# PolyChord/PolyChordLite

Measured on AMD Instinct MI355X. Metric: likelihood evals/sec, 20D Gaussian nlive=2000, higher is better.
Workload: dtype f64; 1 GPU; configs[1]: 20-D Gaussian, nlive=2000, num_repeats=40, one full run per step; batch_chains=1000, parallelism=repeat-sharded x1, mode=one run at a time per GPU; R runs in step: roofline.in_step

## Files before the change

polychordlite_amd/csrc/pc_update.hip:

```cpp
#include "pc_state.h"
#include "pc_launch.h"
#include "pc_upd_flag.h"
#include <atomic>
#include <cstdio>
#include <cstdlib>


__device__ __forceinline__ void upd_stage_masked(const double *src0, unsigned long long mask, unsigned long long mmask, double *dst,
                                                 double *tile, int TS, const double *sh, int D, int nT, int lane)
{
    const int ne = dst ? nT : D + 1;
    int n = 0;
    while (mask) {
        int idx[16], cnt = 0;
#pragma unroll
        for (int u = 0; u < 16; ++u) {
            idx[u] = 0;
            if (mask) { idx[u] = __ffsll((long long)mask) - 1; mask &= mask - 1; cnt = u + 1; }
        }
        for (int e = lane; e < ne; e += 64) {
            double v[16];
#pragma unroll
            for (int u = 0; u < 16; ++u) if (u < cnt) v[u] = (e < nT) ? src0[(size_t)idx[u] * nT + e] : 0.0;
            if (dst) {
#pragma unroll
                for (int u = 0; u < 16; ++u) if (u < cnt) dst[(size_t)(n + u) * nT + e] = v[u];
            }
            if (e <= D) {
                const double s = e < D ? sh[e] : 0.0;
#pragma unroll
                for (int u = 0; u < 16; ++u)
                    if (u < cnt && ((mmask >> idx[u]) & 1ull))
                        tile[(size_t)__popcll(mmask & ((1ull << idx[u]) - 1ull)) * TS + e] = e < D ? v[u] - s : 1.0;
            }
        }
        n += cnt;
    }
}

__global__ __launch_bounds__(UPD_NT) void k_upd_flag(PcState S, int nph, unsigned char *keep, int *blk_count, int def, int nblk) { upd_flag_body<false>(S, nph, keep, blk_count, def, nblk, (int)blockIdx.x * 4 + (int)(threadIdx.x >> 6)); }
__global__ __launch_bounds__(UPD_NT) void k_upd_flag_many(const PcManyRec *R, int def) { const PcManyView r = pc_many_view(R, blockIdx.y); if ((int)blockIdx.x * 4 >= r.ia[PC_REC_I_BLOCKS]) return; upd_flag_body<false>(r.S, r.ia[PC_REC_I_ROWS], (unsigned char *)r.p[PC_REC_KEEP], (int *)r.p[PC_REC_BLK], def, r.ia[PC_REC_I_BLOCKS], (int)blockIdx.x * 4 + (int)(threadIdx.x >> 6)); }

__device__ __forceinline__ bool upd_ticket_last(int *ctr, int n, int *last_s)
{
    asm volatile("s_waitcnt vmcnt(0)" ::: "memory");
    __syncthreads();
    if (threadIdx.x == 0) {
        const int t = __hip_atomic_fetch_add(ctr, 1, __ATOMIC_RELAXED, __HIP_MEMORY_SCOPE_AGENT);
        const int last = t == n - 1;
        if (last) {
            __builtin_amdgcn_fence(__ATOMIC_ACQUIRE, "agent");
            asm volatile("s_waitcnt vmcnt(0)" ::: "memory");
            __hip_atomic_store(ctr, 0, __ATOMIC_RELAXED, __HIP_MEMORY_SCOPE_AGENT);
        }
        *last_s = last;
    }
    __syncthreads();
    return *last_s != 0;
}
#define UPD_TICKET_FLAG 1
#define UPD_TICKET_FINAL 2
#define UPD_TICKET_GROUP 16

#define UPD_SELF_BLOCKS 4096
__global__ __launch_bounds__(UPD_NT) void k_upd_flag_scan(PcState S, int nph, unsigned char *keep, int *blk, int def, int nblk, int *ctr)
{
    __shared__ int last_s, wsum[4];
    upd_flag_body<false>(S, nph, keep, blk, def, nblk, (int)blockIdx.x * 4 + (int)(threadIdx.x >> 6));
    if (!upd_ticket_last(ctr + UPD_TICKET_FLAG, (int)gridDim.x, &last_s)) return;
    const int tid = threadIdx.x, lane = tid & 63, wv = tid >> 6, i0 = 16 * tid;
    int c[16], s = 0;
#pragma unroll
    for (int u = 0; u < 16; ++u) { c[u] = (i0 + u < nblk) ? blk[i0 + u] : 0; s += c[u]; }
    int inc = s;
#pragma unroll
    for (int o = 1; o < 64; o <<= 1) { const int t = __shfl_up(inc, o); if (lane >= o) inc += t; }
    if (lane == 63) wsum[wv] = inc;
    __syncthreads();
    int run = inc - s;
    for (int x = 0; x < wv; ++x) run += wsum[x];
#pragma unroll
    for (int u = 0; u < 16; ++u) { if (i0 + u < nblk) blk[i0 + u] = run; run += c[u]; }
    if (tid == UPD_NT - 1) ctr[0] = run;
}


__global__ __launch_bounds__(1024) void k_upd_scan(int *cnt, int n, int *total)
{
    __shared__ int wsum[16];
    __shared__ int carry_s;
    const int tid = threadIdx.x, lane = tid & 63, wv = tid >> 6;
    int carry = 0;
    for (int base = 0; base < n; base += 4096) {
        const int i0 = base + 4 * tid;
        int c[4];
#pragma unroll
        for (int u = 0; u < 4; ++u) c[u] = (i0 + u < n) ? cnt[i0 + u] : 0;
        const int s = (c[0] + c[1]) + (c[2] + c[3]);
        int inc = s;
#pragma unroll
        for (int o = 1; o < 64; o <<= 1) { const int t = __shfl_up(inc, o); if (lane >= o) inc += t; }
        if (lane == 63) wsum[wv] = inc;
        __syncthreads();
        int pre = carry;
        for (int x = 0; x < wv; ++x) pre += wsum[x];
        int run = pre + inc - s;
#pragma unroll
        for (int u = 0; u < 4; ++u) { if (i0 + u < n) cnt[i0 + u] = run; run += c[u]; }
        if (tid == 1023) carry_s = pre + inc;
        __syncthreads();
        carry = carry_s;
    }
    if (tid == 0) *total = carry;
}

__global__ __launch_bounds__(UPD_NT) void k_upd_index(int nph, const unsigned char *keep, const int *blk_off, int *idx)
{
    __shared__ int cnt[4];
    const int tid = threadIdx.x, lane = tid & 63, wv = tid >> 6;
    const int j = blockIdx.x * UPD_ROWS + tid;
    const bool km = j < nph && (keep[j] & 2);
    const unsigned long long m = __ballot(km);
    if (lane == 0) cnt[wv] = __popcll(m);
    __syncthreads();
    int off = blk_off[blockIdx.x];
    for (int x = 0; x < wv; ++x) off += cnt[x];
    if (km) idx[off + __popcll(m & ((1ull << lane) - 1ull))] = j;
}

#define UPD_IDX_NT 256
#define UPD_IDX_BLOCKS 16
__device__ __forceinline__ void upd_index_self_body(int nph, const unsigned char *keep, const int *blk_count, int nblk, int *idx, int *total)
{
    __shared__ int part[4];
    const int tid = threadIdx.x, lane = tid & 63, wv = tid >> 6;
    const int sb0 = blockIdx.x * UPD_IDX_BLOCKS;
    int s = 0;
    for (int b = tid; b < sb0; b += UPD_IDX_NT) s += blk_count[b];
#pragma unroll
    for (int o = 32; o >= 1; o >>= 1) s += __shfl_xor(s, o);
    if (lane == 0) part[wv] = s;
    __syncthreads();
    int off = (part[0] + part[1]) + (part[2] + part[3]);
    const int sbw = sb0 + 4 * wv;
    for (int x = sb0; x < sbw && x < nblk; ++x) off += blk_count[x];
    const unsigned long long below = (1ull << lane) - 1ull;
    for (int q = 0; q < 4; ++q) {
        const int sb = sbw + q;
        if (sb >= nblk) return;
        const int j0 = sb * UPD_ROWS + 4 * lane;
        unsigned w = 0;
        if (j0 + 3 < nph) w = *(const unsigned *)(keep + j0);
        else for (int u = 0; u < 4; ++u) if (j0 + u < nph) w |= (unsigned)keep[j0 + u] << (8 * u);
        int pos = off, all = 0;
        bool f[4];
#pragma unroll
        for (int u = 0; u < 4; ++u) {
            f[u] = (w >> (8 * u + 1)) & 1u;
            const unsigned long long m = __ballot(f[u]);
            pos += __popcll(m & below); all += __popcll(m);
        }
#pragma unroll
        for (int u = 0; u < 4; ++u) if (f[u]) { idx[pos] = j0 + u; pos++; }
        off += all;
        if (sb == nblk - 1 && lane == 0) *total = off;
    }
}
__global__ __launch_bounds__(UPD_IDX_NT) void k_upd_index_self(int nph, const unsigned char *keep, const int *blk_count, int nblk, int *idx, int *total) { upd_index_self_body(nph, keep, blk_count, nblk, idx, total); }
__global__ __launch_bounds__(UPD_IDX_NT) void k_upd_index_self_many(const PcManyRec *R) { const PcManyView r = pc_many_view(R, blockIdx.y); if ((int)blockIdx.x * 16 >= r.ia[PC_REC_I_BLOCKS]) return; upd_index_self_body(r.ia[PC_REC_I_ROWS], (const unsigned char *)r.p[PC_REC_KEEP], (const int *)r.p[PC_REC_BLK], r.ia[PC_REC_I_BLOCKS], (int *)r.p[PC_REC_PHC2], (int *)r.p[PC_REC_TOTAL]); }


__device__ __forceinline__ void upd_stage_idx(const double *base, const int *ridx, int cnt, double *tile, int TS, const double *sh, int D, int nT, int lane)
{
    if (cnt <= 0) return;
    int idx[16];
#pragma unroll
    for (int u = 0; u < 16; ++u) idx[u] = u < cnt ? ridx[u] : 0;
    for (int e0 = lane; e0 <= D; e0 += 128) {
        const int e1 = e0 + 64;
        double v0[16], v1[16];
#pragma unroll
        for (int u = 0; u < 16; ++u) if (u < cnt) { v0[u] = e0 < D ? base[(size_t)idx[u] * nT + e0] : 1.0; v1[u] = e1 < D ? base[(size_t)idx[u] * nT + e1] : 1.0; }
        const double s0 = e0 < D ? sh[e0] : 0.0, s1 = e1 < D ? sh[e1] : 0.0;
#pragma unroll
        for (int u = 0; u < 16; ++u) if (u < cnt) { tile[(size_t)u * TS + e0] = v0[u] - s0; if (e1 <= D) tile[(size_t)u * TS + e1] = v1[u] - s1; }
    }
}

#define UPD_FOLD 16
__device__ __forceinline__ void upd_fold_body(const double *part, int nb, int E, double *part2, int g)
{
    for (int e = threadIdx.x; e < E; e += 256) {
        double t[UPD_FOLD];
#pragma unroll
        for (int u = 0; u < UPD_FOLD; ++u) t[u] = (g * UPD_FOLD + u < nb) ? part[(size_t)(g * UPD_FOLD + u) * E + e] : 0.0;
        double s = 0.0;
#pragma unroll
        for (int u = 0; u < UPD_FOLD; ++u) s += t[u];
        upd_store_wt(part2 + (size_t)g * E + e, s);
    }
}
__global__ __launch_bounds__(256) void k_upd_fold(const double *part, int nb, int E, double *part2) { upd_fold_body(part, nb, E, part2, blockIdx.x); }
__global__ __launch_bounds__(256) void k_upd_fold_many(const PcManyRec *R, int nb, int E) { double *part = pc_as_global((double *)R[blockIdx.y].p[PC_REC_PART], R); upd_fold_body(part, nb, E, part + (size_t)nb * E, blockIdx.x); }


__device__ __forceinline__ void upd_final_fold(int nb, const double *part, int E, int nE, double *tot)
{
    for (int e = threadIdx.x; e < nE; e += 256) {
        double s[4] = {0.0, 0.0, 0.0, 0.0};
        for (int k0 = 0; k0 < nb; k0 += 4 * 16) {
            double t[4][16];
#pragma unroll
            for (int h = 0; h < 4; ++h)
#pragma unroll
                for (int u = 0; u < 16; ++u) t[h][u] = (k0 + h + 4 * u < nb) ? part[(size_t)(k0 + h + 4 * u) * E + e] : 0.0;
#pragma unroll
            for (int h = 0; h < 4; ++h)
#pragma unroll
                for (int u = 0; u < 16; ++u) s[h] += t[h][u];
        }
        tot[e] = (s[0] + s[1]) + (s[2] + s[3]);
    }
    __syncthreads();
}
#define UPD_FINAL_LDS (544 + 1024 + 1024 + 32 + 1)
template <int DMAX>
__device__ __forceinline__ void upd_final_stage(const PcState &S, double *lds, double *shift, int def)
{
    double *tot = lds, *A = tot + 544, *L = A + 1024, *mu = L + 1024;
    int *bad = (int *)(mu + 32);
    const int tid = threadIdx.x, D = S.D, npair = D * (D + 1) / 2;
#ifdef UPD_DBG
    const long long f0 = clock64();
#endif
    if (tid == 0) *bad = 0;
    const double n = tot[npair + D];
    if (tid < D) mu[tid] = tot[npair + tid] / n;
    __syncthreads();
    for (int p = tid; p < D * D; p += 256) {
        const int a = p / D, b = p % D, lo = a < b ? a : b, hi = a < b ? b : a;
        const int idx = lo * D - lo * (lo - 1) / 2 + (hi - lo);
        const double c = n > 1.0 ? tot[idx] / n - mu[lo] * mu[hi] : 0.0;
        A[p] = c; L[p] = 0.0;
        S.cov[p] = c;
    }
    __syncthreads();
#ifdef UPD_DBG
    const long long f1 = clock64();
#endif
    if (tid < 64) {
        double a[DMAX];
#pragma unroll
        for (int k = 0; k < DMAX; ++k) a[k] = (tid < D && k < D) ? A[tid * D + k] : 0.0;
        bool fail = false;
#pragma unroll
        for (int i = 0; i < DMAX; ++i) {
            if (i < D && !fail) {
                const double aii = readlane_f64(a[i], i);
                if (aii <= 0.0) fail = true;
                else {
                    const double lii = sqrt(aii);
                    const double lji = (tid == i) ? lii : a[i] / lii;
                    if (tid >= i) a[i] = lji;
#pragma unroll
                    for (int k = i + 1; k < DMAX; ++k) { const double lki = readlane_f64(lji, k); if (tid > i) a[k] -= lji * lki; }
                }
            }
        }
        if (fail) { if (tid == 0) *bad = 1; }
        else if (tid < D) {
#pragma unroll
            for (int k = 0; k < DMAX; ++k) if (k < D) L[tid * D + k] = (k <= tid) ? a[k] : 0.0;
        }
    }
    __syncthreads();
    if (*bad) {
        double tr = 0.0;
        for (int k = 0; k < D; ++k) tr += A[k * D + k];
        for (int p = tid; p < D * D; p += 256) L[p] = (p / D == p % D) ? sqrt(tr) : 0.0;
        __syncthreads();
    }
    for (int p = tid; p < D * D; p += 256) S.chol[p] = L[p];
    if (tid < D) shift[tid] += mu[tid];
    if (tid == 0) { if (!(def && S.ctl->upd_keep_thr)) S.death_thr[0] = -PC_HUGE; if (def) S.ctl->upd_pending = 0; }
#ifdef UPD_DBG
    if (tid == 0) { const long long f2 = clock64(); S.ctl->gen_cyc[2] += f1 - f0; S.ctl->gen_cyc[3] += f2 - f1; S.ctl->nn_walks += f0; }
#endif
}
template <int NT>
__device__ __forceinline__ void upd_final_body(const PcState &S, int nb, const double *part, int E, double *lds, double *shift, int def)
{
    const int D = S.D;
    upd_final_fold(nb, part, E, D * (D + 1) / 2 + D + 1, lds);
    if (NT != 2 && D <= 8) upd_final_stage<8>(S, lds, shift, def);
    else if (D <= 16) upd_final_stage<16>(S, lds, shift, def);
    else if (NT != 1 && D <= 24) upd_final_stage<24>(S, lds, shift, def);
    else if (NT != 1) upd_final_stage<32>(S, lds, shift, def);
}
__global__ __launch_bounds__(256) void k_upd_final(PcState S, int nb, const double *part, int E, double *shift, int def) { __shared__ double lds[UPD_FINAL_LDS]; upd_final_body<0>(S, nb, part, E, lds, shift, def); }
__global__ __launch_bounds__(256) void k_upd_final_many(const PcManyRec *R, int nb, int E, int def, int G) { __shared__ double lds[UPD_FINAL_LDS]; const PcManyView r = pc_many_view(R, blockIdx.y); upd_final_body<0>(r.S, nb, (const double *)r.p[PC_REC_PART] + (size_t)G * E, E, lds, (double *)r.p[PC_REC_SHIFT], def); }


typedef double upd_v4d __attribute__((ext_vector_type(4)));
template <int NT, int W>
__device__ __forceinline__ void updg_accumulate(const double *tile, int TS, int n16, int wv, int li, int lk, upd_v4d (&acc)[(NT <= 2) ? NT * (NT + 1) / 2 : (NT * (NT + 1) / 2 + 3) / 4])
{
    if constexpr (NT <= 2) {
        for (int q0 = 4 * wv; q0 < n16; q0 += 16) {
            const double *row = tile + (size_t)(q0 + lk) * TS + li;
            double x[NT];
#pragma unroll
            for (int t = 0; t < NT; ++t) x[t] = row[16 * t];
            int q = 0;
#pragma unroll
            for (int ti = 0; ti < NT; ++ti)
#pragma unroll
                for (int tj = ti; tj < NT; ++tj, ++q) acc[q] = __builtin_amdgcn_mfma_f64_16x16x4f64(x[ti], x[tj], acc[q], 0, 0, 0);
        }
    } else {
        for (int ks = 0; ks < (n16 >> 2); ++ks) {
            const double *row = tile + (size_t)(4 * ks + lk) * TS + li;
            double x[NT];
#pragma unroll
            for (int t = 0; t < NT; ++t) x[t] = row[16 * t];
            int q = 0;
#pragma unroll
            for (int ti = 0; ti < NT; ++ti)
#pragma unroll
                for (int tj = ti; tj < NT; ++tj, ++q)
                    if ((q & 3) == W) acc[q >> 2] = __builtin_amdgcn_mfma_f64_16x16x4f64(x[ti], x[tj], acc[q >> 2], 0, 0, 0);
        }
    }
}
__device__ __forceinline__ int updg_slot(int D, int ti, int tj, int li, int lk, int r)
{
    const int a = 16 * ti + lk + 4 * r, b = 16 * tj + li, npair = D * (D + 1) / 2;
    if (a > b || b > D) return -1;
    return (b < D) ? a * D - a * (a - 1) / 2 + (b - a) : (a < D ? npair + a : npair + D);
}

template <int NT, bool IDX, bool CHAIN>
__device__ __forceinline__ void upd_gather_body(const PcState &S, int nph, int nblk, const unsigned char *keep, const int *blk_off,
                                                double *ph2, double *phL2, unsigned *phC2, unsigned long long *phU2,
                                                const int *idx, const int *nidx_p,
                                                const double *shift, double *part, int E, int def, int nlb, int ndb, double *shift_out = nullptr, int *ctr = nullptr)
{
    static_assert(!CHAIN || IDX, "the chain is pool mode's");
    extern __shared__ __attribute__((aligned(16))) char smem[];
    constexpr bool KS = NT <= 2;
    constexpr int TS = KS ? 16 * NT + 1 : 16 * NT + ((NT & 1) ? 0 : 16);
    constexpr int CAP = KS ? 128 : 64;
    constexpr int NACC = KS ? NT * (NT + 1) / 2 : (NT * (NT + 1) / 2 + 3) / 4;
    __shared__ unsigned long long m64[4], mm64[4];
    __shared__ int dix[256];
    const int tmark = def ? S.ctl->upd_tmark : 0x7fffffff, nph0u = def ? S.ctl->upd_nph0 : 0x7fffffff, updT = def ? S.ctl->upd_T : 0;
    const int tid = threadIdx.x, lane = tid & 63, wv = tid >> 6, li = lane & 15, lk = lane >> 4, D = S.D, nT = S.nT;
    constexpr bool pool = IDX;
    double *tile = (double *)smem;
    double *sh = tile + (size_t)CAP * TS;
    for (int d = tid; d < D; d += 256) sh[d] = shift[d];
    for (int e = tid; e < CAP * TS; e += 256) tile[e] = 0.0;
    upd_v4d acc[NACC];
#pragma unroll
    for (int t = 0; t < NACC; ++t) acc[t] = upd_v4d{0.0, 0.0, 0.0, 0.0};
    int nfill = 0;
#ifdef UPD_DBG
    const long long g0 = clock64();
#endif
    auto flush = [&]() __attribute__((always_inline)) {
        __syncthreads();
        const int n16 = (nfill + 15) & ~15;
        for (int e = tid; e < (n16 - nfill) * (D + 1); e += 256) tile[(size_t)(nfill + e / (D + 1)) * TS + e % (D + 1)] = 0.0;
        __syncthreads();
        if (KS || wv == 0) updg_accumulate<NT, 0>(tile, TS, n16, wv, li, lk, acc);
        else if (wv == 1) updg_accumulate<NT, 1>(tile, TS, n16, wv, li, lk, acc);
        else if (wv == 2) updg_accumulate<NT, 2>(tile, TS, n16, wv, li, lk, acc);
        else updg_accumulate<NT, 3>(tile, TS, n16, wv, li, lk, acc);
        __syncthreads();
        nfill = 0;
    };
    auto piece = [&](const double *src, int sub, double *dst) __attribute__((always_inline)) {
        const unsigned long long ms = m64[sub], mms = mm64[sub], below = (1ull << (16 * wv)) - 1ull;
        const int cnt = __popcll(mms);
        if (cnt == 0 && (dst == nullptr || ms == 0ull)) return;
        if (nfill + cnt > CAP) flush();
        upd_stage_masked(src + (size_t)(sub * 64 + 16 * wv) * nT, ((dst ? ms : mms) >> (16 * wv)) & 0xFFFFull, (mms >> (16 * wv)) & 0xFFFFull,
                         dst ? dst + (size_t)__popcll(ms & below) * nT : nullptr, tile + (size_t)(nfill + __popcll(mms & below)) * TS, TS, sh, D, nT, lane);
        nfill += cnt;
    };
    if constexpr (IDX) {
        const int nidx = *nidx_p;
        const int gchunk = (int)gridDim.x - nlb - ndb;
        if constexpr (CHAIN) {
            __shared__ int off_s[UPD_SELF_BLOCKS + 1], ridx_s[2][64];
            const bool mine = (int)blockIdx.x < gchunk && (int)blockIdx.x * 64 < nidx;
            if (mine) {
                for (int b = tid; b < nblk; b += 256) off_s[b] = blk_off[b];
                if (tid == 0) off_s[nblk] = nidx;
                __syncthreads();
            }
            const unsigned long long below = (1ull << lane) - 1ull;
            int par = 0;
            for (int c = blockIdx.x; mine && c * 64 < nidx; c += gchunk, par ^= 1) {
                const int p0 = c * 64, have = min(64, nidx - p0), p1 = p0 + have;
                if (nfill + have > CAP) flush();
                int lo = 0, hi = nblk - 1;
                while (lo < hi) { const int mid = (lo + hi + 1) >> 1; if (off_s[mid] <= p0) lo = mid; else hi = mid - 1; }
                for (int sb = lo + wv; sb < nblk; sb += 4) {
                    const int o = off_s[sb];
                    if (o >= p1) break;
                    if (off_s[sb + 1] == o) continue;
                    const int j0 = sb * UPD_ROWS + 4 * lane;
                    unsigned w = 0;
                    if (j0 + 3 < nph) w = *(const unsigned *)(keep + j0);
                    else for (int u = 0; u < 4; ++u) if (j0 + u < nph) w |= (unsigned)keep[j0 + u] << (8 * u);
                    int pos = o;
                    bool f[4];
#pragma unroll
                    for (int u = 0; u < 4; ++u) { f[u] = (w >> (8 * u + 1)) & 1u; pos += __popcll(__ballot(f[u]) & below); }
#pragma unroll
                    for (int u = 0; u < 4; ++u) if (f[u]) { if (pos >= p0 && pos < p1) ridx_s[par][pos - p0] = j0 + u; pos++; }
                }
                __syncthreads();
                upd_stage_idx(S.phantom, ridx_s[par] + 16 * wv, min(16, have - 16 * wv), tile + (size_t)(nfill + 16 * wv) * TS, TS, sh, D, nT, lane);
                nfill += have;
            }
        } else
        for (int c = blockIdx.x; (int)blockIdx.x < gchunk && c * 64 < nidx; c += gchunk) {
            const int have = min(64, nidx - c * 64);
            if (nfill + have > CAP) flush();
            upd_stage_idx(S.phantom, idx + c * 64 + 16 * wv, min(16, have - 16 * wv), tile + (size_t)(nfill + 16 * wv) * TS, TS, sh, D, nT, lane);
            nfill += have;
        }
    }
    const int total = nblk + nlb + ndb;
    for (int b = IDX ? ((int)blockIdx.x >= (int)gridDim.x - nlb - ndb ? nblk + (int)blockIdx.x - ((int)gridDim.x - nlb - ndb) : total) : blockIdx.x; b < total; b += gridDim.x) {
        __syncthreads();
        if (b < nblk) {
            const int j = b * 256 + tid;
            const bool k = (j < nph) && keep[j];
            const bool km = k && (j < nph0u || (pool ? updT - 1 - (j - nph0u) / S.nr : (j - nph0u) / S.nr) < tmark);
            const unsigned long long m = __ballot(k), mm = __ballot(km);
            if (lane == 0) { m64[wv] = m; mm64[wv] = mm; }
            __syncthreads();
            int off = 0;
            if (!pool) {
                off = blk_off[b];
                for (int x = 0; x < wv; ++x) off += __popcll(m64[x]);
                if (k) {
                    const int pos = off + __popcll(m & ((1ull << lane) - 1ull));
                    phL2[pos] = S.ph_logL[j]; phC2[pos] = S.ph_cuid[j]; phU2[pos] = S.ph_uid[j];
                }
                off = blk_off[b];
            }
            const double *src = S.phantom + (size_t)b * 256 * nT;
            for (int sub = 0; sub < 4; ++sub) {
                piece(src, sub, pool ? nullptr : ph2 + (size_t)off * nT);
                off += __popcll(m64[sub]);
            }
        } else if (b < nblk + nlb) {
            const int r0 = (b - nblk) * 256, r = r0 + tid;
            const bool k = (r < S.Ncap) && S.live_cluster[r] == 0 && (!def || S.slot_step[r] < tmark);
            const unsigned long long m = __ballot(k);
            if (lane == 0) { m64[wv] = m; mm64[wv] = m; }
            __syncthreads();
            const double *src = S.live + (size_t)r0 * nT;
            for (int sub = 0; sub < 4; ++sub) piece(src, sub, nullptr);
        } else {
            const PcCtl *ctl = S.ctl;
            const int T = ctl->upd_T, ts = ctl->upd_ts;
            const int t = tmark + (b - nblk - nlb) * 256 + tid;
            int di = -1;
            if (t < ts) {
                const PcPlan *pw = S.plan + (T - 1 - t);
                const int src = pw->dead_src;
                const bool existed = src >= 0 || (T - 1 - (-src - 1)) < tmark;
                if (pw->dead_idx >= 0 && pw->logw > S.logzero && existed) di = pw->dead_idx;
            }
            const unsigned long long m = __ballot(di >= 0);
            if (di >= 0) dix[wv * 64 + __popcll(m & ((1ull << lane) - 1ull))] = (int)di;
            if (lane == 0) m64[wv] = m;
            __syncthreads();
            for (int sub = 0; sub < 4; ++sub) {
                const int cnt = __popcll(m64[sub]);
                if (cnt == 0) continue;
                if (nfill + cnt > CAP) flush();
                upd_stage_idx(S.dead, dix + sub * 64 + 16 * wv, min(16, cnt - 16 * wv), tile + (size_t)(nfill + 16 * wv) * TS, TS, sh, D, nT, lane);
                nfill += cnt;
            }
        }
    }
#ifdef UPD_DBG
    const long long g1 = clock64();
#endif
    flush();
    double *out = part + (size_t)blockIdx.x * E;
    if constexpr (KS) {
        double *wres = tile;
#pragma unroll
        for (int t = 0; t < NACC; ++t)
#pragma unroll
            for (int r = 0; r < 4; ++r) wres[((size_t)wv * NACC + t) * 256 + (lk + 4 * r) * 16 + li] = acc[t][r];
        __syncthreads();
        if (wv == 0) {
            int q = 0;
#pragma unroll
            for (int ti = 0; ti < NT; ++ti)
#pragma unroll
                for (int tj = ti; tj < NT; ++tj, ++q)
#pragma unroll
                    for (int r = 0; r < 4; ++r) {
                        const int p = updg_slot(D, ti, tj, li, lk, r), idx = (lk + 4 * r) * 16 + li;
                        if (p >= 0) upd_store_wt(out + p, (wres[(size_t)(0 * NACC + q) * 256 + idx] + wres[(size_t)(1 * NACC + q) * 256 + idx]) +
                                              (wres[(size_t)(2 * NACC + q) * 256 + idx] + wres[(size_t)(3 * NACC + q) * 256 + idx]));
                    }
        }
    } else {
        int q = 0;
#pragma unroll
        for (int ti = 0; ti < NT; ++ti)
#pragma unroll
            for (int tj = ti; tj < NT; ++tj, ++q)
                if ((q & 3) == wv) {
#pragma unroll
                    for (int r = 0; r < 4; ++r) { const int p = updg_slot(D, ti, tj, li, lk, r); if (p >= 0) out[p] = acc[q >> 2][r]; }
                }
    }
#ifdef UPD_DBG
    if (IDX && tid == 0) {
        const int gch = (int)gridDim.x - nlb - ndb, kind = (int)blockIdx.x < gch ? 0 : ((int)blockIdx.x < gch + nlb ? 1 : 2);
        atomicAdd((unsigned long long *)&S.ctl->wave_cyc[kind], (unsigned long long)(g1 - g0));
        atomicAdd((unsigned long long *)&S.ctl->wave_cyc[3], (unsigned long long)(clock64() - g1));
    }
#endif
    if constexpr (CHAIN && KS) {
        static_assert(sizeof(double) * UPD_FINAL_LDS <= sizeof(double) * 4 * 3 * 256, "the final stage's LDS fits the row tile");
        __shared__ int last_s;
        const int G = gridDim.x, g = blockIdx.x / UPD_FOLD, ng = (G + UPD_FOLD - 1) / UPD_FOLD;
        double *part2 = part + (size_t)G * E;
        if (!upd_ticket_last(ctr + UPD_TICKET_GROUP + g, min(UPD_FOLD, G - g * UPD_FOLD), &last_s)) return;
        upd_fold_body(part, G, E, part2, g);
        if (!upd_ticket_last(ctr + UPD_TICKET_FINAL, ng, &last_s)) return;
        upd_final_body<NT>(S, ng, part2, E, tile, shift_out, def);
    }
}
template <int NT, bool IDX>
__global__ __launch_bounds__(256) void k_upd_gather(PcState S, int nph, int nblk, const unsigned char *keep, const int *blk_off,
                                                    double *ph2, double *phL2, unsigned *phC2, unsigned long long *phU2,
                                                    const int *idx, const int *nidx_p,
                                                    const double *shift, double *part, int E, int def, int nlb, int ndb)
{ upd_gather_body<NT, IDX, false>(S, nph, nblk, keep, blk_off, ph2, phL2, phC2, phU2, idx, nidx_p, shift, part, E, def, nlb, ndb); }
template <int NT>
__global__ __launch_bounds__(256) void k_upd_chain(PcState S, int nph, int nblk, const unsigned char *keep, const int *blk_off, double *shift, double *part, int E, int def, int nlb, int ndb, int *ctr)
{ upd_gather_body<NT, true, true>(S, nph, nblk, keep, blk_off, nullptr, nullptr, nullptr, nullptr, nullptr, ctr, shift, part, E, def, nlb, ndb, shift, ctr); }
template <int NT>
__global__ __launch_bounds__(256) void k_upd_gather_many(const PcManyRec *R, int E, int def, int nlb, int ndb)
{
    const PcManyView r = pc_many_view(R, blockIdx.y);
    upd_gather_body<NT, true, false>(r.S, r.ia[PC_REC_I_ROWS], r.ia[PC_REC_I_BLOCKS], (const unsigned char *)r.p[PC_REC_KEEP], (const int *)r.p[PC_REC_BLK], (double *)r.p[PC_REC_PH2], (double *)r.p[PC_REC_PHL2], (unsigned *)r.p[PC_REC_PHC2],
                              (unsigned long long *)r.p[PC_REC_PHU2], (const int *)r.p[PC_REC_PHC2], (const int *)r.p[PC_REC_TOTAL], (const double *)r.p[PC_REC_SHIFT], (double *)r.p[PC_REC_PART], E, def, nlb, ndb);
}


__global__ __launch_bounds__(1024) void k_upd_final_w(PcState S, int nb, const double *part, int E, double *shift, int def, double *ncov, int *count)
{
    extern __shared__ __attribute__((aligned(16))) char smem[];
    double *tot = (double *)smem;
    __shared__ double mu[128];
    const int tid = threadIdx.x, D = S.D, npair = D * (D + 1) / 2, nE = npair + D + 1;
    for (int e = tid; e < nE; e += 1024) {
        double s = 0.0;
        for (int k = 0; k < nb; k += 8) {
            double t[8];
#pragma unroll
            for (int u = 0; u < 8; ++u) t[u] = (k + u < nb) ? part[(size_t)(k + u) * E + e] : 0.0;
#pragma unroll
            for (int u = 0; u < 8; ++u) s += t[u];
        }
        tot[e] = s;
    }
    __syncthreads();
    const double n = tot[npair + D];
    if (tid < D) mu[tid] = tot[npair + tid] / n;
    __syncthreads();
    for (int p = tid; p < D * D; p += 1024) {
        const int a = p / D, b = p % D, lo = a < b ? a : b, hi = a < b ? b : a;
        ncov[p] = n > 1.0 ? tot[lo * D - lo * (lo - 1) / 2 + (hi - lo)] - n * mu[lo] * mu[hi] : 0.0;
    }
    if (tid < D) shift[tid] += mu[tid];
    if (tid == 0) { count[0] = (int)n; if (!(def && S.ctl->upd_keep_thr)) S.death_thr[0] = -PC_HUGE; if (def) S.ctl->upd_pending = 0; }
}

static int upd_grid(const PcState *S, int nph, int deferred)
{
    const int nblk = (nph + UPD_ROWS - 1) / UPD_ROWS, nlb = (S->Ncap + UPD_ROWS - 1) / UPD_ROWS, ndb = deferred ? (S->B + UPD_ROWS - 1) / UPD_ROWS : 0;
    static const int cap_env = std::getenv("PC_UPD_GRID") ? std::atoi(std::getenv("PC_UPD_GRID")) : 0;
    const int cap = cap_env > 0 ? cap_env : (S->D < 32 ? 384 : 512);
    if (S->pool) { const int nch = (nph + 63) / 64; return (nch < cap ? (nch > 0 ? nch : 1) : cap) + nlb + ndb; }
    const int total = nblk + nlb + ndb;
    return total < cap ? total : cap;
}

extern "C" int pc_update_fused_ok(const PcState *S, int nc) { return nc == 1 && S->D <= 128; }
extern "C" int pc_update_fused_blocks(const PcState *S, int nph)
{
    const int G = upd_grid(S, nph, 1), E = pc_update_fused_entries(S);
    return G + (G + UPD_FOLD - 1) / UPD_FOLD + (S->D * S->D + 2 + E - 1) / E;
}
extern "C" int pc_update_fused_entries(const PcState *S) { const int e = S->D * (S->D + 1) / 2 + S->D + 1; return (e + 31) & ~31; }

extern "C" void pc_launch_update_fused(const PcState *S, int nph, unsigned char *keep, int *blk, int *d_total, double *ph2, double *phL2,
                                       unsigned *phC2, unsigned long long *phU2, double *part, double *shift, int deferred, hipStream_t st)
{
    pc_launch_update_fused_at(S, nph, keep, blk, d_total, ph2, phL2, phC2, phU2, part, shift, deferred, 0, st);
}
extern "C" void pc_launch_update_fused_at(const PcState *S, int nph, unsigned char *keep, int *blk, int *d_total, double *ph2, double *phL2,
                                          unsigned *phC2, unsigned long long *phU2, double *part, double *shift, int deferred, int flagged, hipStream_t st)
{
    const int D = S->D, nblk = (nph + UPD_ROWS - 1) / UPD_ROWS, nlb = (S->Ncap + UPD_ROWS - 1) / UPD_ROWS, E = pc_update_fused_entries(S);
    const int ndb = deferred ? (S->B + UPD_ROWS - 1) / UPD_ROWS : 0;
    const int NTv = (D + 1 + 15) / 16, TSv = NTv <= 2 ? 16 * NTv + 1 : 16 * NTv + ((NTv & 1) ? 0 : 16), CAPv = NTv <= 2 ? 128 : 64;
    const int G = upd_grid(S, nph, deferred), ng = (G + UPD_FOLD - 1) / UPD_FOLD;
    double *part2 = part + (size_t)G * E;
    size_t shw = sizeof(double) * ((size_t)CAPv * TSv + D);
    if (NTv <= 2 && shw < sizeof(double) * (size_t)(4 * 3 * 256)) shw = sizeof(double) * (size_t)(4 * 3 * 256);
    if (S->pool && nblk <= UPD_SELF_BLOCKS && UPD_TICKET_GROUP + ng <= PC_UPD_CTR_INTS && (S->ablate & PC_ABL_UPDATE_CHAIN)) {
        int *ctr = d_total;
        hipLaunchKernelGGL(k_upd_flag_scan, dim3((nblk + 3) / 4), dim3(UPD_NT), 0, st, *S, nph, keep, blk, deferred, nblk, ctr);
#define UPDC_LAUNCH(NT) { \
        pc_need_dyn_lds((const void *)k_upd_chain<NT>, shw); \
        hipLaunchKernelGGL((k_upd_chain<NT>), dim3(G), dim3(256), shw, st, *S, nph, nblk, (const unsigned char *)keep, (const int *)blk, shift, part, E, deferred, nlb, ndb, ctr); }
        switch (NTv) { case 1: UPDC_LAUNCH(1) break; case 2: UPDC_LAUNCH(2) break; case 3: UPDC_LAUNCH(3) break; case 4: UPDC_LAUNCH(4) break;
                       case 5: UPDC_LAUNCH(5) break; case 6: UPDC_LAUNCH(6) break; case 7: UPDC_LAUNCH(7) break; case 8: UPDC_LAUNCH(8) break;
                       default: UPDC_LAUNCH(9) break; }
#undef UPDC_LAUNCH
        if (D < 32) return;
    } else {
        if (!(flagged && S->pool && deferred)) hipLaunchKernelGGL(k_upd_flag, dim3((nblk + 3) / 4), dim3(UPD_NT), 0, st, *S, nph, keep, blk, deferred, nblk);
        if (!S->pool) pc_launch_scan_blocks(blk, nblk, d_total, &S->ctl->nphantom, st);
        else if (nblk <= UPD_SELF_BLOCKS && !std::getenv("PC_UPD_SCAN_LAUNCH"))
            hipLaunchKernelGGL(k_upd_index_self, dim3((nblk + 15) / 16), dim3(UPD_IDX_NT), 0, st, nph, (const unsigned char *)keep, (const int *)blk, nblk, (int *)phC2, d_total);
        else {
            hipLaunchKernelGGL(k_upd_scan, dim3(1), dim3(1024), 0, st, blk, nblk, d_total);
            hipLaunchKernelGGL(k_upd_index, dim3(nblk), dim3(UPD_NT), 0, st, nph, (const unsigned char *)keep, (const int *)blk, (int *)phC2);
        }
        int devi = 0; (void)hipGetDevice(&devi); devi &= 63;
#define UPDG_LAUNCH(NT) { \
            pc_need_dyn_lds((const void *)k_upd_gather<NT, false>, shw); \
                              pc_need_dyn_lds((const void *)k_upd_gather<NT, true>, shw); \
             \
            if (S->pool) hipLaunchKernelGGL((k_upd_gather<NT, true>), dim3(G), dim3(256), shw, st, *S, nph, nblk, (const unsigned char *)keep, (const int *)blk, \
                               ph2, phL2, phC2, phU2, (const int *)phC2, (const int *)d_total, (const double *)shift, part, E, deferred, nlb, ndb); \
            else hipLaunchKernelGGL((k_upd_gather<NT, false>), dim3(G), dim3(256), shw, st, *S, nph, nblk, (const unsigned char *)keep, (const int *)blk, \
                               ph2, phL2, phC2, phU2, (const int *)nullptr, (const int *)nullptr, (const double *)shift, part, E, deferred, nlb, ndb); }
        switch (NTv) { case 1: UPDG_LAUNCH(1) break; case 2: UPDG_LAUNCH(2) break; case 3: UPDG_LAUNCH(3) break; case 4: UPDG_LAUNCH(4) break;
                       case 5: UPDG_LAUNCH(5) break; case 6: UPDG_LAUNCH(6) break; case 7: UPDG_LAUNCH(7) break; case 8: UPDG_LAUNCH(8) break;
                       default: UPDG_LAUNCH(9) break; }
#undef UPDG_LAUNCH
    }
    hipLaunchKernelGGL(k_upd_fold, dim3(ng), dim3(256), 0, st, (const double *)part, G, E, part2);
    if (D < 32) { hipLaunchKernelGGL(k_upd_final, dim3(1), dim3(256), 0, st, *S, ng, (const double *)part2, E, shift, deferred); return; }
    double *ncov = part2 + (size_t)ng * E;
    int *count = (int *)(ncov + (size_t)D * D);
    const size_t shf = sizeof(double) * (size_t)(D * (D + 1) / 2 + D + 1);
    pc_need_dyn_lds((const void *)k_upd_final_w, shf);
    hipLaunchKernelGGL(k_upd_final_w, dim3(1), dim3(1024), shf, st, *S, ng, (const double *)part2, E, shift, deferred, ncov, count);
    pc_launch_chol_only(S, ncov, count, st);
}

extern "C" int pc_update_fused_grid(const PcState *S, int nph, int deferred) { return upd_grid(S, nph, deferred); }
extern "C" int pc_launch_update_fused_many(const PcState *S, const PcManyRec *dR, int R, int nblk_max, int G, int deferred, hipStream_t st)
{
    const int D = S->D, nlb = (S->Ncap + UPD_ROWS - 1) / UPD_ROWS, E = pc_update_fused_entries(S);
    if (!S->pool || nblk_max > UPD_SELF_BLOCKS || D >= 32 || nblk_max < 1) return 1;
    const int ndb = deferred ? (S->B + UPD_ROWS - 1) / UPD_ROWS : 0;
    const int NTv = (D + 1 + 15) / 16, TSv = NTv <= 2 ? 16 * NTv + 1 : 16 * NTv + ((NTv & 1) ? 0 : 16), CAPv = NTv <= 2 ? 128 : 64;
    const int ng = (G + UPD_FOLD - 1) / UPD_FOLD;
    size_t shw = sizeof(double) * ((size_t)CAPv * TSv + D);
    if (NTv <= 2 && shw < sizeof(double) * (size_t)(4 * 3 * 256)) shw = sizeof(double) * (size_t)(4 * 3 * 256);
    hipLaunchKernelGGL(k_upd_flag_many, dim3((nblk_max + 3) / 4, R), dim3(UPD_NT), 0, st, dR, deferred);
    hipLaunchKernelGGL(k_upd_index_self_many, dim3((nblk_max + 15) / 16, R), dim3(UPD_IDX_NT), 0, st, dR);
    int devi = 0; (void)hipGetDevice(&devi); devi &= 63;
#define UPDM_LAUNCH(NT) { \
        pc_need_dyn_lds((const void *)k_upd_gather_many<NT>, shw); \
        hipLaunchKernelGGL((k_upd_gather_many<NT>), dim3(G, R), dim3(256), shw, st, dR, E, deferred, nlb, ndb); }
    if (NTv == 1) UPDM_LAUNCH(1) else UPDM_LAUNCH(2)
#undef UPDM_LAUNCH
    hipLaunchKernelGGL(k_upd_fold_many, dim3(ng, R), dim3(256), 0, st, dR, G, E);
    hipLaunchKernelGGL(k_upd_final_many, dim3(1, R), dim3(256), 0, st, dR, ng, E, deferred, G);
    return 0;
}
```

Baseline: 1.365 billion likelihood evals/s.

## Prefetch gather indices and batch multi-chunk row loads in update gather

Hoists the keep-word and block-count loads in the index-compaction kernel ahead of the block reduction, so their latency overlaps the prefix sum. In the pool gather path, each wave now issues loads for up to four 64-row chunks at once into registers, with the next chunk's indices fetched in between. The shift and tile writes happen afterwards. The live and dead staging paths get the same batched loading for small tile counts. This targets memory latency in the gather, at the cost of much higher register pressure and more complex index clamping.

```diff
diff --git a/polychordlite_amd/csrc/pc_update.hip b/polychordlite_amd/csrc/pc_update.hip
--- a/polychordlite_amd/csrc/pc_update.hip
+++ b/polychordlite_amd/csrc/pc_update.hip
@@ -135,6 +135,20 @@
     __shared__ int part[4];
     const int tid = threadIdx.x, lane = tid & 63, wv = tid >> 6;
     const int sb0 = blockIdx.x * UPD_IDX_BLOCKS;
+    const int sbw = sb0 + 4 * wv;
+    unsigned w4[4];
+#pragma unroll
+    for (int q = 0; q < 4; ++q) {
+        const int j0 = (sbw + q) * UPD_ROWS + 4 * lane;
+        w4[q] = 0;
+        if (sbw + q < nblk) {
+            if (j0 + 3 < nph) w4[q] = *(const unsigned *)(keep + j0);
+            else for (int u = 0; u < 4; ++u) if (j0 + u < nph) w4[q] |= (unsigned)keep[j0 + u] << (8 * u);
+        }
+    }
+    int front[UPD_IDX_BLOCKS - 4];
+#pragma unroll
+    for (int x = 0; x < UPD_IDX_BLOCKS - 4; ++x) front[x] = (x < 4 * wv && sb0 + x < nblk) ? blk_count[sb0 + x] : 0;
     int s = 0;
     for (int b = tid; b < sb0; b += UPD_IDX_NT) s += blk_count[b];
 #pragma unroll
@@ -142,16 +156,15 @@
     if (lane == 0) part[wv] = s;
     __syncthreads();
     int off = (part[0] + part[1]) + (part[2] + part[3]);
-    const int sbw = sb0 + 4 * wv;
-    for (int x = sb0; x < sbw && x < nblk; ++x) off += blk_count[x];
+#pragma unroll
+    for (int x = 0; x < UPD_IDX_BLOCKS - 4; ++x) off += front[x];
     const unsigned long long below = (1ull << lane) - 1ull;
+#pragma unroll
     for (int q = 0; q < 4; ++q) {
         const int sb = sbw + q;
         if (sb >= nblk) return;
         const int j0 = sb * UPD_ROWS + 4 * lane;
-        unsigned w = 0;
-        if (j0 + 3 < nph) w = *(const unsigned *)(keep + j0);
-        else for (int u = 0; u < 4; ++u) if (j0 + u < nph) w |= (unsigned)keep[j0 + u] << (8 * u);
+        const unsigned w = w4[q];
         int pos = off, all = 0;
         bool f[4];
 #pragma unroll
@@ -339,6 +352,7 @@
     return (b < D) ? a * D - a * (a - 1) / 2 + (b - a) : (a < D ? npair + a : npair + D);
 }
 
+#define UPD_AHEAD(NT) ((NT) <= 3 ? 4 : ((NT) <= 8 ? 2 : 1))
 template <int NT, bool IDX, bool CHAIN>
 __device__ __forceinline__ void upd_gather_body(const PcState &S, int nph, int nblk, const unsigned char *keep, const int *blk_off,
                                                 double *ph2, double *phL2, unsigned *phC2, unsigned long long *phU2,
@@ -358,6 +372,17 @@
     constexpr bool pool = IDX;
     double *tile = (double *)smem;
     double *sh = tile + (size_t)CAP * TS;
+    constexpr bool AHEAD = IDX && !CHAIN && UPD_AHEAD(NT) > 1;
+    const int gchunk = (int)gridDim.x - nlb - ndb;
+    auto ask = [&](long long c0) __attribute__((always_inline)) {
+        const long long p = (c0 + (long long)min(lane >> 4, UPD_AHEAD(NT) - 1) * gchunk) * 64 + 16 * wv + (lane & 15);
+        return idx[p < (long long)nph ? p : (long long)nph - 1];
+    };
+    int nidx_v = 0, rnext = 0;
+    if constexpr (AHEAD) {
+        nidx_v = __hip_atomic_load(nidx_p, __ATOMIC_RELAXED, __HIP_MEMORY_SCOPE_AGENT);
+        if ((int)blockIdx.x < gchunk) rnext = ask(blockIdx.x);
+    }
     for (int d = tid; d < D; d += 256) sh[d] = shift[d];
     for (int e = tid; e < CAP * TS; e += 256) tile[e] = 0.0;
     upd_v4d acc[NACC];
@@ -388,9 +413,38 @@
                          dst ? dst + (size_t)__popcll(ms & below) * nT : nullptr, tile + (size_t)(nfill + __popcll(mms & below)) * TS, TS, sh, D, nT, lane);
         nfill += cnt;
     };
+    auto ahead = [&](const double *base, int rows, const auto &have, const auto &off, const auto &cnt, auto between) __attribute__((always_inline)) {
+        constexpr int K = sizeof(have) / sizeof(int);
+        constexpr bool TWO = NT > 4;
+        const int e0 = lane, e1 = lane + 64;
+        double v0[K][16], v1[TWO ? K : 1][16];
+#pragma unroll
+        for (int k = 0; k < K; ++k)
+#pragma unroll
+            for (int u = 0; u < 16; ++u)
+                if (u < cnt[k]) {
+                    const double *row = base + (size_t)__builtin_amdgcn_readlane(rows, 16 * k + u) * nT;
+                    v0[k][u] = e0 < D ? row[e0] : 1.0;
+                    if constexpr (TWO) v1[k][u] = e1 < D ? row[e1] : 1.0;
+                }
+        between();
+        const double s0 = e0 < D ? sh[e0] : 0.0, s1 = (TWO && e1 < D) ? sh[e1] : 0.0;
+#pragma unroll
+        for (int k = 0; k < K; ++k) {
+            if (have[k] <= 0) continue;
+            if (nfill + have[k] > CAP) flush();
+            double *trow = tile + (size_t)(nfill + off[k]) * TS;
+            if (e0 <= D) {
+#pragma unroll
+                for (int u = 0; u < 16; ++u) if (u < cnt[k]) { trow[(size_t)u * TS + e0] = v0[k][u] - s0; if constexpr (TWO) { if (e1 <= D) trow[(size_t)u * TS + e1] = v1[k][u] - s1; } }
+            }
+            nfill += have[k];
+        }
+    };
     if constexpr (IDX) {
-        const int nidx = *nidx_p;
-        const int gchunk = (int)gridDim.x - nlb - ndb;
+        int nidx;
+        if constexpr (AHEAD) { __syncthreads(); nidx = __builtin_amdgcn_readfirstlane(nidx_v); }
+        else nidx = *nidx_p;
         if constexpr (CHAIN) {
             __shared__ int off_s[UPD_SELF_BLOCKS + 1], ridx_s[2][64];
             const bool mine = (int)blockIdx.x < gchunk && (int)blockIdx.x * 64 < nidx;
@@ -425,12 +479,27 @@
                 upd_stage_idx(S.phantom, ridx_s[par] + 16 * wv, min(16, have - 16 * wv), tile + (size_t)(nfill + 16 * wv) * TS, TS, sh, D, nT, lane);
                 nfill += have;
             }
-        } else
-        for (int c = blockIdx.x; (int)blockIdx.x < gchunk && c * 64 < nidx; c += gchunk) {
-            const int have = min(64, nidx - c * 64);
-            if (nfill + have > CAP) flush();
-            upd_stage_idx(S.phantom, idx + c * 64 + 16 * wv, min(16, have - 16 * wv), tile + (size_t)(nfill + 16 * wv) * TS, TS, sh, D, nT, lane);
-            nfill += have;
+        } else if constexpr (UPD_AHEAD(NT) == 1) {
+            for (int c = blockIdx.x; (int)blockIdx.x < gchunk && c * 64 < nidx; c += gchunk) {
+                const int have = min(64, nidx - c * 64);
+                if (nfill + have > CAP) flush();
+                upd_stage_idx(S.phantom, idx + c * 64 + 16 * wv, min(16, have - 16 * wv), tile + (size_t)(nfill + 16 * wv) * TS, TS, sh, D, nT, lane);
+                nfill += have;
+            }
+        } else {
+            constexpr int K = UPD_AHEAD(NT);
+            const bool mine = (int)blockIdx.x < gchunk;
+            for (long long c = blockIdx.x; mine && c * 64 < nidx; c += (long long)K * gchunk) {
+                const int rcur = min(max(rnext, 0), nph - 1);
+                int have[K], off[K], cnt[K];
+#pragma unroll
+                for (int k = 0; k < K; ++k) {
+                    const long long left = (long long)nidx - (c + (long long)k * gchunk) * 64;
+                    have[k] = (int)max(0ll, min(64ll, left)); off[k] = 16 * wv; cnt[k] = have[k] - 16 * wv;
+                }
+                const bool more = (c + (long long)K * gchunk) * 64 < nidx;
+                ahead(S.phantom, rcur, have, off, cnt, [&]() __attribute__((always_inline)) { if (more) rnext = ask(c + (long long)K * gchunk); });
+            }
         }
     }
     const int total = nblk + nlb + ndb;
@@ -465,6 +534,18 @@
             if (lane == 0) { m64[wv] = m; mm64[wv] = m; }
             __syncthreads();
             const double *src = S.live + (size_t)r0 * nT;
+            if constexpr (IDX && UPD_AHEAD(NT) == 4) {
+                int have[4], off[4], cnt[4];
+#pragma unroll
+                for (int k = 0; k < 4; ++k) {
+                    const unsigned long long mk = (unsigned long long)(unsigned)__builtin_amdgcn_readfirstlane((unsigned)m64[k]) | ((unsigned long long)(unsigned)__builtin_amdgcn_readfirstlane((unsigned)(m64[k] >> 32)) << 32);
+                    have[k] = __popcll(mk); off[k] = __popcll(mk & ((1ull << (16 * wv)) - 1ull)); cnt[k] = __popcll((mk >> (16 * wv)) & 0xFFFFull);
+                }
+                unsigned mw = (unsigned)(m64[lane >> 4] >> (16 * wv)) & 0xFFFFu;
+                for (int x = 0; x < (lane & 15); ++x) mw &= mw - 1u;
+                const int rows = (lane >> 4) * 64 + 16 * wv + (mw ? __ffs((int)mw) - 1 : 0);
+                ahead(src, rows, have, off, cnt, []() {});
+            } else
             for (int sub = 0; sub < 4; ++sub) piece(src, sub, nullptr);
         } else {
             const PcCtl *ctl = S.ctl;
@@ -481,6 +562,17 @@
             if (di >= 0) dix[wv * 64 + __popcll(m & ((1ull << lane) - 1ull))] = (int)di;
             if (lane == 0) m64[wv] = m;
             __syncthreads();
+            if constexpr (IDX && UPD_AHEAD(NT) == 4) {
+                int have[4], off[4], cnt[4];
+#pragma unroll
+                for (int k = 0; k < 4; ++k) {
+                    have[k] = __popc(__builtin_amdgcn_readfirstlane((unsigned)m64[k])) + __popc(__builtin_amdgcn_readfirstlane((unsigned)(m64[k] >> 32)));
+                    off[k] = 16 * wv; cnt[k] = have[k] - 16 * wv;
+                }
+                const int mine = min(max(__popcll(m64[lane >> 4]) - 16 * wv, 0), 16);
+                const int rows = (lane & 15) < mine ? dix[(lane >> 4) * 64 + 16 * wv + (lane & 15)] : 0;
+                ahead(S.dead, rows, have, off, cnt, []() {});
+            } else
             for (int sub = 0; sub < 4; ++sub) {
                 const int cnt = __popcll(m64[sub]);
                 if (cnt == 0) continue;
```

Result: no change. 1.369 billion likelihood evals/s, median of 6 (+0.3%).
